# areanddee/Sharding-the-Sphere-Fall-2025-JAX-DevLab-Examples

Hardware: AMD Instinct MI355X
Metric: cell-updates/sec (whole node) at C96 (higher is better)
Workload: dtype fp64; 1 GPU; global_batch=1, seq_len=55296, parallelism=spatial tiles: 24 tiles over 1 GPU(s), auto partition, N=96, tiles_per_edge=2, integrator=ssprk3, backend=hip, comm=none, steps_per_launch=6, fused_block=16, graph_replayed_steps=0, direct_launch_steps=1662, kernel_launches=277, eager_steps=0

## Files before the change

### sharding-the-sphere-fall-2025-jax-devlab-examples_amd/ops/build.py

```python
from __future__ import annotations

import argparse
import os
import subprocess
import sys

HERE = os.path.dirname(os.path.abspath(__file__))
CSRC = os.path.join(HERE, "csrc")
LIB = os.path.join(HERE, "libstsp.so")
SOURCES = ["stage_kernel.hip", "march_kernel.hip", "march3_kernel.hip", "swe_tracer_stage.hip", "fused_step.hip", "derived_kernel.hip", "latlon_kernel.hip", "points_kernel.hip", "spectra_kernel.hip", "synth_kernel.hip", "tt_kernels.hip", "tt_persist.hip", "runtime.cpp"]
HEADERS = ["stsp_kernels.h", "stage_common.h", "xg_ring.h", "xg_codec.h", "march_common.h", "tt_common.h", "runtime.h", "rccl_abi.h"]
ARCH = os.environ.get("STSP_OFFLOAD_ARCH", "gfx950")
VARIANT_FLAGS = {"": [], "diag": ["-DSTSP_STAMPS"],
                 "unfused": ["-DSTSP_FUSE_FACES=0"], "pe0": ["-DSTSP_PE_WAVE=0"],
                 "ownw0": ["-DSTSP_OWN_SKIP0=0"], "w9": ["-DSTSP_W10=0"], "swsqrt": ["-DSTSP_HW_SQRT=0"],
                 "selslope": ["-DSTSP_SIGN_SLOPE=0"], "wpe6": ["-DSTSP_WPE=6"], "wpe7": ["-DSTSP_WPE=7"],
                 "fp_alledge": ["-DSTSP_FPROBE_ALLEDGE=1"],
                 "xgfence": ["-DSTSP_XG_FENCE=1"],
                 "hrt0": ["-DSTSP_FUSED_TAIL_OWN=0", "-DSTSP_FUSED_POLL2=0", "-DSTSP_FUSED_RF_MINB=1000"],
                 "hrt1": ["-DSTSP_FUSED_POLL2=0", "-DSTSP_FUSED_RF_MINB=1000"],
                 "hrt12": ["-DSTSP_FUSED_RF_MINB=1000"]}


def lib_for(variant: str = "") -> str:
    return LIB if not variant else os.path.join(HERE, f"libstsp_{variant}.so")


def _hipcc() -> str:
    for c in (os.environ.get("HIPCC"), "/opt/rocm/bin/hipcc", "hipcc"):
        if c and (os.path.exists(c) or c == "hipcc"):
            return c
    raise RuntimeError("hipcc not found")


def needs_build(variant: str = "") -> bool:
    lib = lib_for(variant)
    if not os.path.exists(lib):
        return True
    t = os.path.getmtime(lib)
    for f in SOURCES + HEADERS:
        p = os.path.join(CSRC, f)
        if os.path.exists(p) and os.path.getmtime(p) > t:
            return True
    return False


def _obj_dir(variant: str) -> str:
    return os.path.join(HERE, "_obj", variant or "prod")


def build(force: bool = False, verbose: bool = False, variant: str = "") -> str:
    lib = lib_for(variant)
    if not force and not needs_build(variant):
        return lib
# ... 56 lines not shown
```

### sharding-the-sphere-fall-2025-jax-devlab-examples_amd/ops/csrc/fused_step.hip

```cpp
#include "stage_common.h"

#include <type_traits>


#ifndef STSP_FPROBE_ALLEDGE
#define STSP_FPROBE_ALLEDGE 0
#endif
#ifndef STSP_XG_FENCE
#define STSP_XG_FENCE 0
#endif
#ifndef STSP_FUSED_TAGH
#define STSP_FUSED_TAGH 1
#endif
#ifndef STSP_FUSED_TAIL_OWN
#define STSP_FUSED_TAIL_OWN 1
#endif
#ifndef STSP_FUSED_POLL2
#define STSP_FUSED_POLL2 1
#endif
#ifndef STSP_FUSED_RF_MINB
#define STSP_FUSED_RF_MINB 12
#endif

namespace {

constexpr int CT_INTS = 16, CT_FLAGS = 12, CG_VALS = 8;

template <int NS, int B>
struct FD {
  static constexpr int R = 2 * NS;
  static constexpr int W = B + 2 * R;
  static constexpr int WS = W + 1;
  static constexpr int GMAX = 160;
  static constexpr int GB = W * WS;
  static constexpr int WW = GB + GMAX;
  static constexpr int L1 = R - 2 * (NS - 1);
  static constexpr int H1 = B + 4 * (NS - 1);
  static constexpr int NFX = H1 * (H1 + 1);
  static constexpr int NFL = 2 * NFX;
  static constexpr int NU = H1 * H1;
  static constexpr int NT = NU <= 768 ? 768 : 1024;
  static_assert(NU <= NT && W * W <= 2 * NT, "owner threads for every updated cell");
  static constexpr int NTAIL = W * W > NT ? W * W - NT : 0;
  static constexpr int NTO = STSP_FUSED_TAIL_OWN ? B * B : NT - NU;
  static constexpr int TPT = NTAIL ? (NTAIL + NTO - 1) / NTO : 1;
  static_assert(GMAX <= NT, "one fix-up thread per ghost entry");
  static_assert(2 * (B + 4 * (NS - 2)) * (B + 4 * (NS - 2) + 1) <= 32 * 64 && 2 * H1 * (H1 + 1) <= 32 * 64 + 64 * 64,
                "face passes per stage fit the 32-entry pass table");
  static constexpr int CMAX = 32;
};

__device__ __forceinline__ int fregion(int X, int Y, int N) {
  const bool inx = (unsigned)X < (unsigned)N, iny = (unsigned)Y < (unsigned)N;
  if (inx) return iny ? 0 : (Y < 0 ? 3 : 4);
  return iny ? (X < 0 ? 1 : 2) : -1;
}

__host__ __device__ __forceinline__ constexpr void annulus(int t, int lo, int L, int w, int& u, int& v) {
  if (t < w * L) {
    u = lo + t % L; v = lo + t / L;
    return;
  }
  t -= w * L;
  if (t < w * L) {
    u = lo + t % L; v = lo + L - w + t / L;
    return;
  }
  t -= w * L;
  const int r = t / (2 * w), c = t - r * 2 * w;
  v = lo + w + r;
  u = c < w ? lo + c : lo + L - 2 * w + c;
}

template <int NS, int B>
__host__ __device__ __forceinline__ constexpr void owner_cell(int t, int& u, int& v) {
  using D = FD<NS, B>;
  constexpr int R = D::R;
  if (t < B * B) {
    u = R + t % B; v = R + t / B;
    return;
  }
  int done = B * B;
#pragma unroll
  for (int k = 1; k <= NS; ++k) {
    const int L = B + 4 * k;
    const int n = L * L - (L - 4) * (L - 4);
    if (t < done + n) {
      annulus(t - done, R - 2 * k, L, 2, u, v);
      return;
    }
    done += n;
  }
  u = -1; v = -1;
}

template <int NS, int B>
__host__ __device__ __forceinline__ constexpr int tail_index(int tid, int k) {
  using D = FD<NS, B>;
  if (!D::NTAIL || k >= D::TPT) return -1;
  const int first = STSP_FUSED_TAIL_OWN ? 0 : D::NU;
  if (tid < first || tid >= first + D::NTO) return -1;
  const int idx = D::NT + (tid - first) + k * D::NTO;
  return idx < D::W * D::W ? idx : -1;
}

template <int NS, int B>
constexpr bool window_covered_once() {
  using D = FD<NS, B>;
  constexpr int W = D::W;
  int cnt[W * W] = {};
  for (int t = 0; t < D::NT; ++t) {
    int idx[1 + D::TPT] = {};
    idx[0] = t < W * W ? t : -1;
    for (int k = 0; k < D::TPT; ++k) idx[1 + k] = tail_index<NS, B>(t, k);
    for (int k = 0; k <= D::TPT; ++k) {
      if (idx[k] < 0) continue;
      if (k > 0 && idx[k] < D::NT) return false;
      int u = -1, v = -1;
      owner_cell<NS, B>(idx[k], u, v);
      if (u < 0 || u >= W || v < 0 || v >= W) return false;
      ++cnt[v * W + u];
    }
  }
  for (int c = 0; c < W * W; ++c)
    if (cnt[c] != 1) return false;
  return true;
}

template <typename T>
struct FArgs {
  const T* Q;
  T* out;
  const int* src;
  const int* org;
  const T* len;
  const T* nrm;
  const T* tane;
  const T* crec;
  const T* lxt;
  const T* gbt;
  unsigned long long frames;
  const unsigned long long* code;
  const int* gtab;
  const T* gw;
  const int* ctab;
  const T* cgf;
  const int* ccnt;
  const int* push;
  const int* cpush;
  int G, C, nblocks, n, N, S, mg, pw;
  int links[6];
  int local_src;
  unsigned mdiv_n;
  T a0[4], a1[4], a2[4];
  T dt, g, omega2;
  int ring, K;
  const unsigned long long* recv;
  T* const* peer_ring;
  const int* xpush;
  int* epoch;
// ... 97 lines not shown
  if (fr & 64) xi = -xi;
  if (fr & 128) xj = -xj;
  if (fr & 256) xn = -xn;
  o0 = ai == 0 ? xi : (aj == 0 ? xj : xn);
  o1 = ai == 1 ? xi : (aj == 1 ? xj : xn);
  o2 = ai == 2 ? xi : (aj == 2 ? xj : xn);
}

template <typename T>
__device__ __forceinline__ T pair_swap(T v) {
  if constexpr (sizeof(T) == 8) {
    int2 p = __builtin_bit_cast(int2, v);
    p.x = __builtin_amdgcn_update_dpp(0, p.x, 0xB1, 0xF, 0xF, false);
    p.y = __builtin_amdgcn_update_dpp(0, p.y, 0xB1, 0xF, 0xF, false);
    return __builtin_bit_cast(T, p);
  } else {
    return __builtin_bit_cast(T, __builtin_amdgcn_update_dpp(0, __builtin_bit_cast(int, v), 0xB1, 0xF, 0xF, false));
  }
}

__device__ __forceinline__ int sel5(int r, int v0, int v1, int v2, int v3, int v4) {
  return r == 0 ? v0 : r == 1 ? v1 : r == 2 ? v2 : r == 3 ? v3 : v4;
}

__device__ __forceinline__ int ncode(unsigned long long c, int side) {
  return (int)(short)(unsigned short)(c >> (16 * side));
}

template <typename T, int LIM, int NS, int B, bool XG, bool MULTI>
__global__ __launch_bounds__((FD<NS, B>::NT)) void fused_step_kernel(FArgs<T> a) {
  using D = FD<NS, B>;
  constexpr int W = D::W, WS = D::WS, WW = D::WW, GB = D::GB, R = D::R, L1 = D::L1, H1 = D::H1;
  constexpr int NFX = D::NFX, NFL = D::NFL, NT = D::NT;
  static_assert(window_covered_once<NS, B>(), "owner and tail cells cover the window exactly once");
  constexpr bool RING_FIRST = B >= STSP_FUSED_RF_MINB;
  constexpr bool PFN = sizeof(T) == 4 || B <= 16;
  constexpr int NRG = PFN ? 1 : 5;
  constexpr int NN = 2 * NRG * 3 * (W + 1);
  __shared__ T s_w[5 * WW];
  __shared__ T s_fl[4][NFL];
  __shared__ T s_len[NFL];
  __shared__ T s_nrm[2][NRG][3][W + 1];
  __shared__ T s_nrmf[PFN ? 3 * NFL : 1];
  constexpr int CS = W + 1;
  __shared__ unsigned long long s_code[W * CS];
  __shared__ short s_gs[D::GMAX][2];
  __shared__ T s_gt[D::GMAX];
  __shared__ int s_ct[D::CMAX][CT_INTS];
  __shared__ T s_cg[D::CMAX][CG_VALS];
  constexpr int NX2 = NS > 1 ? (B + 4 * (NS - 2)) * (B + 4 * (NS - 2)) : 1;
  __shared__ T s_x[4][NX2];
  __shared__ int s_gdone;

  const int tid = threadIdx.x;
  const int bid = xcd_remap(blockIdx.x, a.nblocks);
  const int N = a.N;
  const int* og = a.org + bid * 4;
  const int X0 = og[0], Y0 = og[1], tile = og[2], ow = og[3];
  const int xo = ow & 0xFFF, yo = (ow >> 12) & 0xFFF, flags = (ow >> 24) & 0x1F;
  const bool edge = (flags & 0x1E) != 0;
  const int ngw = edge ? (a.G + 63) >> 6 : 0;
  int gbase = 0;
  int gtarget = 0;
  if (tid == 0) s_gdone = 0;
  const T* wf = &s_w[0];
  FSTAMP(0);
  FSTAMP_RT(14);
  if (a.stamps && (tid & 63) == 0) {
    unsigned long long* sp = a.stamps + ((long)bid * 16 + (tid >> 6)) * FST_W;
    sp[16] = __builtin_amdgcn_s_getreg((31 << 11) | 4);
    sp[17] = __builtin_amdgcn_s_getreg((31 << 11) | 20);
    sp[18] = blockIdx.x;
  }

  int u = -1, v = -1;
  const bool owner = tid < W * W;
  if (owner) owner_cell<NS, B>(tid, u, v);
  const int wi = v * WS + u;
  int xe = 0;
  const int nsteps = MULTI ? a.nsteps : 1;
  const bool epoch_on = XG || MULTI;
  const bool tagh = STSP_FUSED_TAGH && MULTI && a.hx != nullptr;
  const bool pcell = MULTI && !XG && !tagh && a.pidx != nullptr;
  if (epoch_on) xe = a.epoch[bid];
  const int n = a.n;
  const int face0 = (int)((unsigned)ow >> 29);
  auto cell_src = [&](int cu, int cv, int& g_, int& I_, int& J_) -> int {
    if (!window_cell(face0, X0 + cu, Y0 + cv, N, a.links, g_, I_, J_)) return -1;
    if (a.local_src) {
      const int t = N / n;
      const int ti = a.mdiv_n ? (int)__umulhi((unsigned)I_, a.mdiv_n) : I_ / n;
      const int tj = a.mdiv_n ? (int)__umulhi((unsigned)J_, a.mdiv_n) : J_ / n;
      return (((g_ * t + tj) * t + ti) * a.pw + (J_ - tj * n) + a.mg) * a.pw + (I_ - ti * n) + a.mg;
    }
    return a.src[(long)bid * W * W + cv * W + cu];
  };
  int cg_ = 0, cI = 0, cJ = 0;
  const int src = owner ? cell_src(u, v, cg_, cI, cJ) : -1;
  unsigned long long cdv = 0;
  int gs0 = 0, gs1 = 0;
  T gtv = T(0);
  int ncor = 0;
  int ctv[CT_INTS];
  T cgv[CG_VALS];
  if (edge) {
    if (owner) cdv = a.code[(long)bid * W * W + v * W + u];
    if (tid < a.G) {
      gs0 = a.gtab[((long)bid * a.G + tid) * 2];
      gs1 = a.gtab[((long)bid * a.G + tid) * 2 + 1];
// ... 28 lines not shown
      const int r = yf ? jj / H1 : jj / (H1 + 1), c = yf ? jj - r * H1 : jj - r * (H1 + 1);
      const int li = yf ? (X0 + L1 + c) * (N + 1) + Y0 + L1 + r : (Y0 + L1 + r) * (N + 1) + X0 + L1 + c;
      lnv[k] = j < NFL ? a.lxt[li] : T(0);
    }
  } else {
#pragma unroll
    for (int k = 0; k < LPT; ++k) {
      const int j = tid + k * NT;
      lnv[k] = j < NFL ? a.len[(long)bid * NFL + j] : T(0);
    }
  }
  T nrv = T(0);
  const bool nr_ld = flags == 1 ? tid < 2 * (W + 1) : (!PFN && tid < NN);
  T nrv2 = T(0);
  if (nr_ld) {
    if (flags == 1) nrv = a.tane[(tid < W + 1 ? X0 + tid : Y0 + tid - (W + 1))];
    else nrv = a.nrm[(long)bid * NN + tid];
  }
  static_assert(NN <= 2 * NT, "line-normal table: two values per thread at most");
  if (!PFN && NN > NT && flags != 1 && tid + NT < NN) nrv2 = a.nrm[(long)bid * NN + tid + NT];
  constexpr int NPF = PFN ? (3 * NFL + NT - 1) / NT : 1;
  T nfv[NPF];
  if (PFN && flags != 1) {
#pragma unroll
    for (int k = 0; k < NPF; ++k) {
      const int j = tid + k * NT;
      nfv[k] = j < 3 * NFL ? a.nrmf[(long)bid * 3 * NFL + j] : T(0);
    }
  }
  T Q[4];
  T iA = T(0), r0 = T(0), r1 = T(0), r2 = T(0), gb0 = T(0), gb1 = T(0), gb2 = T(0), S0 = T(0), S1 = T(0),
    S2 = T(0);
  const bool loaded = src >= 0 || (XG && src <= -2);
  const bool in1 = tid < (B + 4 * (NS - 1)) * (B + 4 * (NS - 1));
  auto load_state_of = [&](int src, T (&Q)[4], const T* Qin, int xe_) {
    const bool loaded = src >= 0 || (XG && src <= -2);
    if (XG && src <= -2) {
      unsigned long long gr[HX<T>::W];
      const XgRec r = ring_slot_record<HX<T>>(a.recv, a.ring, xg_in_slot(xe_), -2 - src);
      fused_wait<HX<T>, XG_RING_SCOPE, STSP_XG_FENCE != 0>(r, xg_in_tag(xe_), a.err, a.timeout_ticks, gr, [&] {
        fused_fail(a.err, 1u, bid, xe_, -2 - src, (int)HX<T>::tag_of(gr[0]));
      });
      HX<T>::unpack(gr, Q);
    } else if (loaded) {
      const unsigned S = (unsigned)a.S;
      unsigned so = (unsigned)src;
      asm volatile("" : "+v"(so));
#pragma unroll
      for (int f = 0; f < 4; ++f) Q[f] = ld_state<true>(o32(Qin, so + f * S));
    } else {
#pragma unroll
      for (int f = 0; f < 4; ++f) Q[f] = T(0);
    }
  };
  auto hx_record = [&](unsigned so, int slot) -> XgRec {
    const unsigned S = (unsigned)a.S;
    return {(gu64*)a.hx + (size_t)slot * HX<T>::W * S + so, (long)S};
  };
  auto load_tagged = [&](int src_, T (&q)[4], int xe_) {
#if STSP_FUSED_TAIL_OWN
    asm volatile("" : "+v"(src_));
#endif
    unsigned long long gr[HX<T>::W];
    const XgRec r = hx_record((unsigned)src_, xe_ & 1);
    fused_wait<HX<T>, XG_LOCAL_SCOPE>(r, xg_in_tag(xe_), a.err, a.timeout_ticks, gr, [&] {
      fused_fail(a.err, 2u, bid, xe_, src_, (int)HX<T>::tag_of(gr[0]));
    });
// ... 286 lines not shown
      tail_load(buf[it & 1], xe, tq);
      if (tid >= B * B) {
        load_state(buf[it & 1], xe);
        enter_cell();
      }
    }
    tail_put(tq);
    FSTAMP(19);
    __syncthreads();
  }
  FSTAMP(2);

#pragma unroll
  for (int s = 0; s < NS; ++s) {
    const int lo = R - 2 * (NS - 1 - s), hi = W - lo;
    const int nr = hi - lo, nl = nr + 1, nx = nr * nl;
    if (edge) {
      const int ge = tid - gbase;
      if (ge >= 0 && ge < a.G) {
        const int i0 = s_gs[ge][0], i1 = s_gs[ge][1];
        const T t = s_gt[ge];
#pragma unroll
        for (int f = 0; f < 4; ++f) {
          const T x0 = wf[f * WW + i0], x1 = wf[f * WW + i1];
          s_w[f * WW + GB + ge] = x0 + t * (x1 - x0);
        }
      }
      if (ge >= 0 && ge < ngw * 64 && (tid & 63) == 0) {
        asm volatile("s_waitcnt lgkmcnt(0)" ::: "memory");
        __hip_atomic_fetch_add(&s_gdone, 1, __ATOMIC_RELEASE, __HIP_MEMORY_SCOPE_WORKGROUP);
      }
      gtarget += ngw;
    }
    const int nax = s == 0 ? NOX : nx;
    const int ntask = 2 * nax;
    unsigned m = pmask[s];
    for (int first = (ncor && wv == 0) ? 1 : 0; first || m;) {
      int task;
      bool nearp = false;
      if (first) {
        task = (tid & 63) - 64;
        first = 0;
      } else {
        const int pp = __builtin_ctz(m);
        task = pp * 64 + (tid & 63);
        nearp = (nmask[s] >> pp) & 1u;
        m &= m - 1u;
      }
      if (task >= ntask) continue;
      if (task >= 0) {
        const int tf = task;
        const bool ax = tf >= nax;
        const int t2 = ax ? tf - nax : tf;
        int fu, fv, k, p;
        if (s == 0) {
          outer_face(t2, k, p);
        } else {
          const int c = t2 / nr, r = t2 - c * nr;
          k = lo + c; p = lo + r;
        }
        if (!ax) { fv = p; fu = k; }
        else { fu = p; fv = k; }
        if (edge || STSP_FPROBE_ALLEDGE) {
          if (PFN && !nearp) face(ax, fu, fv, k, std::integral_constant<int, 1>{});
          else face(ax, fu, fv, k, std::integral_constant<int, 2>{});
        } else {
          face(ax, fu, fv, k, std::integral_constant<int, 0>{});
        }
      } else {
        const int lane = tid & 63, j = lane >> 1, q = lane & 1;
        const bool live = j < ncor;
        T fvq[4], ccq[5];
#pragma unroll
        for (int f = 0; f < 4; ++f) fvq[f] = T(0);
#pragma unroll
        for (int f = 0; f < 5; ++f) ccq[f] = T(0);
        int fl_ = 0;
        if (live) {
          const int* ct = s_ct[j];
          fl_ = ct[CT_FLAGS];
          const int ic = ct[5 * q], a0 = ct[5 * q + 1], a1 = ct[5 * q + 2], n0 = ct[5 * q + 3], n1 = ct[5 * q + 4];
          const bool plus = (fl_ >> (4 + q)) & 1, ai = (fl_ >> (2 * q)) & 1, ni = (fl_ >> (2 * q + 1)) & 1;
          const T ta = s_cg[j][4 + 2 * q], tn = s_cg[j][5 + 2 * q];
#pragma unroll
          for (int f = 0; f < 5; ++f) ccq[f] = wf[f * WW + ic];
#pragma unroll
          for (int f = 0; f < 4; ++f) {
            const T c0 = ccq[f];
            const T xa = wf[f * WW + a0], xn = wf[f * WW + n0];
            const T across = ai ? xa + ta * (wf[f * WW + a1] - xa) : xa;
            const T inward = ni ? xn + tn * (wf[f * WW + n1] - xn) : xn;
            fvq[f] = plus ? c0 + half_slope<LIM>(c0 - inward, across - c0)
                          : c0 - half_slope<LIM>(c0 - across, inward - c0);
          }
        }
        T fvp[4], ccp[5];
#pragma unroll
        for (int f = 0; f < 4; ++f) fvp[f] = pair_swap(fvq[f]);
#pragma unroll
        for (int f = 0; f < 5; ++f) ccp[f] = pair_swap(ccq[f]);
        if (live && q == 0) {
          T fl[4];
          swe_flux<T>(fvq, fvp, ccq, ccp, s_cg[j][0], s_cg[j][1], s_cg[j][2], s_cg[j][3], a.g, fl);
          const int fc = s_ct[j][10], fd = s_ct[j][11];
          const bool pc = (fl_ >> 4) & 1, pd = (fl_ >> 5) & 1;
#pragma unroll
          for (int f = 0; f < 4; ++f) {
            if (fc >= 0) s_fl[f][fc] = pc ? fl[f] : -fl[f];
            if (fd >= 0) s_fl[f][fd] = pd ? -fl[f] : fl[f];
          }
        }
      }
    }
    FSTAMP(10 + s);
    __syncthreads();
    FSTAMP(3 + 2 * s);
    const bool upd = loaded && tid < nr * nr;
    if (upd) {
      const int xw = (v - L1) * (H1 + 1) + (u - L1), xe_ = xw + 1;
      const int ys = NFX + (v - L1) * H1 + (u - L1), yn = ys + H1;
      T dq[4];
#pragma unroll
      for (int f = 0; f < 4; ++f) dq[f] = -((s_fl[f][xe_] - s_fl[f][xw]) + (s_fl[f][yn] - s_fl[f][ys])) * iA;
      const T h = Q[0];
      const T fcor = a.omega2 * r2;
      const T cor[3] = {r1 * Q[3] - r2 * Q[2], r2 * Q[1] - r0 * Q[3], r0 * Q[2] - r1 * Q[1]};
      const T pb = T(0.5) * a.g * h * h * iA, gh = a.g * h;
      const T gbv[3] = {gb0, gb1, gb2}, Sv[3] = {S0, S1, S2};
#pragma unroll
      for (int k = 0; k < 3; ++k) dq[1 + k] += -fcor * cor[k] + pb * Sv[k] - gh * gbv[k];
      const T c0 = a.a0[s], c1 = a.a1[s], c2 = a.a2[s] * a.dt;
      T o[4];
#pragma unroll
      for (int f = 0; f < 4; ++f) {
        T base = c1 * Q[f];
        if (c0 != T(0)) base += c0 * s_x[f][tid];
        o[f] = c2 * dq[f] + base;
      }
      const T dd = o[1] * r0 + o[2] * r1 + o[3] * r2;
      o[1] -= dd * r0; o[2] -= dd * r1; o[3] -= dd * r2;
#pragma unroll
      for (int f = 0; f < 4; ++f) Q[f] = o[f];
      if (s + 1 < NS) put(Q);
    }
    if (s + 1 < NS) __syncthreads();
    FSTAMP(4 + 2 * s);
  }

  T* const Out = buf[(it + 1) & 1];
  const bool last = it + 1 == nsteps;
// ... 185 lines not shown
  return -5;
}

template <typename T>
__global__ __launch_bounds__(256) void fused_prime_kernel(const T* __restrict__ q, int S,
                                                          const int* __restrict__ src, const int* __restrict__ code,
                                                          int nent, T* const* peer_ring, int ring, int epoch) {
  const int i = blockIdx.x * blockDim.x + threadIdx.x;
  if (i < nent) {
    xg_prime_record<HX<T>, 4>(q, S, src[i], code[i], peer_ring, ring, epoch);
  }
  __threadfence_system();
}

extern "C" int stsp_fused_record_words(int dtype) { return dtype == 1 ? HX<double>::W : HX<float>::W; }

extern "C" int stsp_fused_prime_launch(int dtype, const void* q, int S, const int* src, const int* code, int nent,
                                       void* const* peer_ring, int ring, int epoch, hipStream_t stream) {
  if (nent <= 0) return 0;
  const dim3 grid((nent + 255) / 256), block(256);
  if (dtype == 1)
    hipLaunchKernelGGL(fused_prime_kernel<double>, grid, block, 0, stream, (const double*)q, S, src, code, nent,
                       (double* const*)peer_ring, ring, epoch);
  else if (dtype == 0)
    hipLaunchKernelGGL(fused_prime_kernel<float>, grid, block, 0, stream, (const float*)q, S, src, code, nent,
                       (float* const*)peer_ring, ring, epoch);
  else
    return -4;
  return (int)hipGetLastError();
}

extern "C" int stsp_fused_tagh(void) { return STSP_FUSED_TAGH; }

extern "C" int stsp_fused_limits(int* gmax, int* cmax) {
  *gmax = FD<3, 16>::GMAX;
  *cmax = FD<3, 16>::CMAX;
  return 0;
}
```

### sharding-the-sphere-fall-2025-jax-devlab-examples_amd/ops/fused.py

```python
from __future__ import annotations

import hashlib
import os
from dataclasses import dataclass
from typing import Dict, List, Optional, Tuple

import numpy as np
import torch

from ..models.base import panel_edge_tables
from ..parallel.layout import TileLayout, ghost_xy
from ..parallel.topology import neighbor_cells


def native_stream(device) -> int:
    from .native import current_stream_handle
    return current_stream_handle(device)

REG_P, REG_W, REG_E, REG_S, REG_N = 0, 1, 2, 3, 4
NREG = 5
SIDE_VEC = ((-1, 0), (1, 0), (0, -1), (0, 1))
NG_PLR = 2


# ... 704 lines not shown
        e.time += e.dt
        e.step_count += 1



FUSED_BLOCKS = (6, 8, 12, 16, 18, 20)


def rank_cus(device) -> int:
    import os
    cus = torch.cuda.get_device_properties(device).multi_processor_count
    if os.environ.get("STSP_SHARE_GPU") == "1":
        cus = max(1, cus // max(1, int(os.environ.get("WORLD_SIZE", "1"))))
    return cus


def fused_block(n: int, tiles: Optional[int] = None, cus: Optional[int] = None) -> Optional[int]:
    fits = [B for B in FUSED_BLOCKS if n % B == 0]
    if not fits:
        return None
    if tiles is not None and cus is not None:
        for B in fits:
            if tiles * (n // B) ** 2 <= cus:
                return B
    return fits[-1]



def fused_threads(B: int, ns: int = 3) -> int:
    h1 = B + 4 * (ns - 1)
    return 768 if h1 * h1 <= 768 else 1024


def stage_face_counts(B: int, ns: int = 3) -> List[int]:
    h1 = B + 4 * (ns - 1)
    nil = B - 3
    out = [2 * (h1 * (h1 + 1) - nil * B)]
    for s in range(1, ns):
        nr = B + 4 * (ns - 1 - s)
        out.append(2 * nr * (nr + 1))
    return out


PASS_SLOTS = 32


def pass_schedule(B: int, ncorner: np.ndarray, edge: np.ndarray, G: int, ns: int = 3,
                  weights: Optional[str] = None) -> np.ndarray:
    import os
    weights = weights or os.environ.get("STSP_FUSED_SCHED", "5:1")
    nt = fused_threads(B, ns)
    nw = nt // 64
    counts = stage_face_counts(B, ns)
    nb = len(ncorner)
    out = np.zeros((nb, ns, PASS_SLOTS), dtype=np.uint8)
    ngw = -(-G // 64) if G > 0 else 0
    cache = {}
    for b in range(nb):
        cw = 1 if ncorner[b] > 0 else 0
        gw = ngw if edge[b] else 0
        key = (cw, gw)
        if key not in cache:
            tab = np.zeros((ns, PASS_SLOTS), dtype=np.uint8)
            for s, nt_s in enumerate(counts):
                npass = -(-nt_s // 64)
                assert npass <= PASS_SLOTS
                if weights == "legacy":
                    first = nw - cw
                    for p in range(npass):
                        tab[s, p] = p + cw if p < first else cw + gw + (p - first) % (nw - cw - gw)
                    continue
                wc, wg = (int(x) for x in weights.split(":"))
                wl = [0] * nw
                if cw:
                    wl[0] += wc
                for w in range(cw, cw + gw):
                    wl[w] += wg
                for p in range(npass):
                    gl = [sum(wl[w] for w in range(g, nw, 4)) for g in range(4)]
                    g = min(range(4), key=lambda g_: (gl[g_], g_))
                    w = min(range(g, nw, 4), key=lambda w_: (wl[w_], w_))
                    tab[s, p] = w
                    wl[w] += 4
            cache[key] = tab
        out[b] = cache[key]
    return out


def pass_masks(B: int, sched: np.ndarray, ns: int = 3, near: Optional[np.ndarray] = None) -> np.ndarray:
    counts = stage_face_counts(B, ns)
    nb = sched.shape[0]
    m = np.zeros((nb, ns, 17), dtype=np.uint32)
    for s_, cnt in enumerate(counts):
        for p in range(-(-cnt // 64)):
            w = sched[:, s_, p].astype(np.int64)
            m[np.arange(nb), s_, w] |= np.uint32(1 << p)
    if near is not None:
        m[:, :, 16] = near
    return m


def stage_face_coords(B: int, ns: int = 3) -> List[Tuple[np.ndarray, np.ndarray, np.ndarray]]:
    d = FusedDims.make(B, ns)
    R, W, L1, H1 = d.R, d.W, d.L1, d.H1
    nil = B - 3
    ol0 = R + 2 - L1
    ol1 = (W - L1) - (R + B - 1) + 1
    nr1, nor = H1, H1 - B
    noa = (ol0 + ol1) * nr1
    nox = noa + nil * nor
    out = []
    for s_ in range(ns):
        if s_ == 0:
            nax = nox
            t = np.arange(nax)
            k = np.empty(nax, np.int64)
            p = np.empty(nax, np.int64)
            a = t < noa
            li, r = np.divmod(t[a], nr1)
            k[a] = np.where(li < ol0, L1 + li, R + B - 1 + (li - ol0))
            p[a] = L1 + r
            t2 = t[~a] - noa
            li, r = np.divmod(t2, nor)
            k[~a] = R + 2 + li
            p[~a] = np.where(r < R - L1, L1 + r, R + B + (r - (R - L1)))
        else:
            lo = R - 2 * (ns - 1 - s_)
            nr = W - 2 * lo
            nax = nr * (nr + 1)
            c, r = np.divmod(np.arange(nax), nr)
            k, p = lo + c, lo + r
        out.append((np.concatenate([np.zeros(nax, np.int64), np.ones(nax, np.int64)]),
                    np.concatenate([k, k]), np.concatenate([p, p])))
    return out


def near_pass_masks(B: int, org: np.ndarray, flags: np.ndarray, N: int, ns: int = 3) -> np.ndarray:
    nb = org.shape[0]
    out = np.zeros((nb, ns), dtype=np.uint32)
    coords = stage_face_coords(B, ns)
    far = -1000
    X0, Y0 = org[:, 0].astype(np.int64), org[:, 1].astype(np.int64)
    kx0 = np.where(flags & 2, -X0, far)
    kx1 = np.where(flags & 4, N - X0, far)
    ky0 = np.where(flags & 8, -Y0, far)
    ky1 = np.where(flags & 16, N - Y0, far)
    for s_, (ax, k, _) in enumerate(coords):
        e0 = np.where(ax[None, :] == 1, ky0[:, None], kx0[:, None])
        e1 = np.where(ax[None, :] == 1, ky1[:, None], kx1[:, None])
        kk = k[None, :]
        near = ((kk - e0 + 1 >= 0) & (kk - e0 + 1 <= 2)) | ((kk - e1 + 1 >= 0) & (kk - e1 + 1 <= 2))
        npass = -(-near.shape[1] // 64)
        for p in range(npass):
            hit = near[:, 64 * p:64 * (p + 1)].any(1)
            out[hit, s_] |= np.uint32(1 << p)
    return out


def face_normals(P: "FusedPlan", flags: np.ndarray) -> np.ndarray:
    d = P.d
    H1, L1 = d.H1, d.L1
    nfx = d.nfx
    nfl = 2 * nfx
    j = np.arange(nfl)
    yf = j >= nfx
    jj = np.where(yf, j - nfx, j)
    r = np.where(yf, jj // H1, jj // (H1 + 1))
    c = np.where(yf, jj - r * H1, jj - r * (H1 + 1))
    fu = L1 + c
    fv = L1 + r
    k = np.where(yf, fv, fu)
    lu = fu - np.where(yf, 0, 1)
    lv = fv - np.where(yf, 1, 0)
# ... 44 lines not shown
        if why:
            raise RuntimeError(why)
        if B is None:
            cus = None
            if engine.device.type == "cuda":
                cus = rank_cus(engine.device)
            B = fused_block(engine.plan.n, len(engine.plan.tiles), cus)
        e = engine
        self.e = e
        self.group = group
        self.lib = native.require_native()
        self._launch_fn = self.lib.stsp_fused_launch
        world = e.layout.num_ranks
        self.world = world
        X = None
        if world > 1 or e.layout.loopback:
            X = FusedExchangePlan(e.layout, e.grid, B, ns=3)
            P = X.plans[e.rank]
        else:
            P = FusedPlan(e.layout, e.rank, e.grid, B=B, ns=3)
            P.src[~P.need[:, 0]] = -1
        self.plan = P
        d = P.d
        W, WS, nb = d.W, d.W + 1, P.nb
        dev, dt = e.device, e.dtype
        gmax, cmax = ctypes_limits(self.lib)
        G, C = P.gtab.shape[1], P.ctab.shape[1]
        if G > gmax or C > cmax:
            raise RuntimeError(f"fused step: {G} ghost entries / {C} corner faces exceed the kernel's {gmax} / {cmax}")
        S = e.plan.S
        nring = X.ring_slots if X is not None else 0
        assert P.src.shape == (nb, W * W) and int(P.src.max()) < S and int(P.src.min()) >= -2 - (nring - 1)
        assert (P.src[P.need[:, 0]] != -1).all()
        nfl = 2 * d.nfx
        ld = lambda s_: (s_ // W) * WS + s_ % W
        for b in range(nb):
            k = int(P.gcnt[b])
            assert (P.gtab[b, :k, 2:4] >= 0).all() and (P.gtab[b, :k, 2:4] < W * W).all()
            for j in range(int(P.ccnt[b])):
                assert -1 <= P.ctab[b, j, 4] < nfl and -1 <= P.ctab[b, j, 5] < nfl
        assert int(P.gidx.max()) < G
        code = neighbour_codes(P)
        gpair = np.zeros((nb, G, 2), dtype=np.int32)
        gpair[..., 0] = ld(P.gtab[..., 2])
        gpair[..., 1] = ld(P.gtab[..., 3])
        ct, cgw = corner_tables(P, code, gpair)
        org = P.org.copy()
        for b in range(nb):
            regs = set(int(x) for x in np.unique(P.reg[b]) if x >= 0)
            flags = sum(1 << r for r in regs)
            li, rem = divmod(b, P.nbx * P.nby)
            yb, xb = divmod(rem, P.nbx)
            face = e.layout.tile_origin(e.plan.tiles[li])[0]
            org[b, 3] = np.int32(np.uint32((xb * B) | ((yb * B) << 12) | (flags << 24) | (face << 29)).view(np.int32))
        kg = kernel_geometry(e.layout, e.grid)
        self.frames = [int(x) for x in kg["frames"]]
        t = lambda a, ty=dt: torch.as_tensor(np.ascontiguousarray(a), dtype=ty, device=dev)
        self.tens = {
            "len": t(np.concatenate([P.lx.reshape(nb, -1), P.ly.reshape(nb, -1)], 1)),
            "nrm": t(np.ascontiguousarray(np.moveaxis(P.nrm, -1, -2))),
            "tane": t(kg["tane"]), "crec": t(kg["crec"]), "lxt": t(kg["lxt"]),
            "src": t(P.src, torch.int32), "org": t(org, torch.int32),
            "code": t(code.view(np.int64), torch.int64), "gtab": t(gpair, torch.int32), "gw": t(P.gt),
            "ctab": t(ct, torch.int32), "cgf": t(cgw), "ccnt": t(P.ccnt, torch.int32),
            "push": torch.as_tensor(e.plan.push_map, dtype=torch.int32, device=dev).contiguous(),
            "cpush": torch.as_tensor(e.plan.corner_push, dtype=torch.int32, device=dev).contiguous(),
# ... 9 lines not shown
            for li, tid in enumerate(e.plan.tiles):
                f, I0, J0 = L_.tile_origin(tid)
                gbn[li, ng:ng + n, ng:ng + n, :3] = rec_g[L_.global_flat(f, I0 + ii, J0 + jj), 4:7]
            gbn = gbn.reshape(-1, 4)
            if X is not None:
                rg = np.zeros((len(X.need_remote[e.rank]), 4))
                rg[:, :3] = rec_g[X.need_remote[e.rank], 4:7]
                gbn = np.concatenate([gbn, rg], 0)
            self.tens["gbt"] = t(gbn)
        assert int(e.plan.push_map.max(initial=-1)) < S and int(e.plan.corner_push.max(initial=-1)) < S
        self.dcode = native.dtype_code(dt)
        self.mem = None
        self.tens["epoch"] = torch.zeros(nb, dtype=torch.int32, device=dev)
        self.handoff = handoff_mode(B, multi_rank=X is not None)
        if self.handoff == "tag" and not read_relation_symmetric(P):
            if os.environ.get("STSP_FUSED_HANDOFF") == "tag":
                raise RuntimeError("tagged hand-off needs a symmetric block read relation")
            self.handoff = "epoch"
        if self.handoff == "tag" and not int(self.lib.stsp_fused_tagh()):
            if os.environ.get("STSP_FUSED_HANDOFF") == "tag":
                raise RuntimeError("STSP_FUSED_HANDOFF=tag needs a library built with STSP_FUSED_TAGH=1")
            self.handoff = "epoch"
        if self.handoff == "tag":
            words = 5 if e.dtype == torch.float64 else 4
            self.tens["hx"] = torch.zeros(2 * words * e.plan.S, dtype=torch.int64, device=dev)
        self.tens["err"] = torch.zeros(8, dtype=torch.int32, device=dev)
        prod = producer_table(P)
        self.tens["prod"] = torch.as_tensor(prod, dtype=torch.int32, device=dev).contiguous()
        self.poll = poll_mode() if (X is None and self.handoff == "epoch" and read_relation_symmetric(P)) \
            else "block"
        if self.poll == "cell":
            self.tens["pidx"] = torch.as_tensor(cell_producer_index(P, prod), device=dev).contiguous()
        edge_b = np.array([any(int(x) > 0 for x in np.unique(P.reg[b])) for b in range(nb)])
        sched = pass_schedule(B, np.asarray(P.ccnt), edge_b, G)
        assert int(sched.max()) < fused_threads(B) // 64
        flg = (org[:, 3].view(np.uint32) >> 24) & 0x1F
        near = near_pass_masks(B, P.org, flg.astype(np.int64), e.layout.N)
        self.tens["sched"] = torch.as_tensor(pass_masks(B, sched, near=near).view(np.int32), device=dev).contiguous()
        self.tens["nrmf"] = t(face_normals(P, flg.astype(np.int64)))
        self.timeout_ticks = int(timeout_s * 1e8)
        if X is not None:
            self._setup_exchange(X, timeout_s)
        self.descs = [self._desc(0, 1), self._desc(1, 0)]
        self._multi = {}
        self._multi_ptrs = {}
        if X is not None:
            self.prime()

    def _setup_exchange(self, X, timeout_s: float) -> None:
        from .xgmi import IpcRing, _declare, refuse_if_forced
        refuse_if_forced()
        e = self.e
        L = _declare(self.lib)
        self._xlib = L
        self.slots = int(L.stsp_xg_slots())
        self.ring = X.ring_slots * int(self.lib.stsp_fused_record_words(self.dcode))
        xpush, psrc, pcode = X.producer(e.rank)
        assert psrc.size == 0 or int(psrc.max()) < e.plan.S
        peers = sorted(set(int(c) >> XG_SLOT_BITS for c in pcode.tolist())
                       | set(int(x) for x in np.unique(np.asarray(e.layout.owner)[
                           e.layout.locate(X.need_remote[e.rank])[0]]).tolist()))
        self.mem = IpcRing(L, e.device, self.world, e.rank, peers, self.slots * self.ring * 8, self.group)
        pr = np.zeros(32, dtype=np.int64)
        for p, b in self.mem.bases.items():
            pr[p] = b
        dev = e.device
        self.tens.update({
            "peer_ring": torch.as_tensor(pr, device=dev),
            "xpush": torch.as_tensor(xpush, dtype=torch.int32, device=dev).contiguous(),
            "prime_src": torch.as_tensor(psrc, dtype=torch.int32, device=dev),
            "prime_code": torch.as_tensor(pcode, dtype=torch.int32, device=dev),
# ... 369 lines not shown
```

### sharding-the-sphere-fall-2025-jax-devlab-examples_amd/ops/native.py

```python
from __future__ import annotations

import ctypes
import os
import threading

import torch

from . import build as _build

_LIB = None
_LOCK = threading.Lock()


class StageDesc(ctypes.Structure):
    _fields_ = [
        ("X", ctypes.c_void_p), ("Q", ctypes.c_void_p), ("acc_in", ctypes.c_void_p),
        ("out", ctypes.c_void_p), ("acc_out", ctypes.c_void_p), ("recv", ctypes.c_void_p),
        ("gmap", ctypes.c_void_p), ("push", ctypes.c_void_p), ("blocks", ctypes.c_void_p),
        ("invA", ctypes.c_void_p), ("ex", ctypes.c_void_p), ("ey", ctypes.c_void_p),
        ("mx", ctypes.c_void_p), ("my", ctypes.c_void_p), ("cgeo", ctypes.c_void_p),
        ("ntile", ctypes.c_int), ("n", ctypes.c_int), ("S", ctypes.c_int), ("mg", ctypes.c_int), ("pw", ctypes.c_int),
        ("nblocks", ctypes.c_int), ("limiter", ctypes.c_int), ("remote", ctypes.c_int),
        ("a0", ctypes.c_double), ("a1", ctypes.c_double), ("a2", ctypes.c_double),
        ("c0", ctypes.c_double), ("c1", ctypes.c_double), ("c2", ctypes.c_double), ("dt", ctypes.c_double),
# ... 115 lines not shown
    ("stsp_synth_launch", [_P(SynthDesc), _VP], SynthDesc, ("stsp_synth_desc_size", ())),
]


def lib_path() -> str:
    return _build.lib_for(os.environ.get("STSP_VARIANT", ""))


def load(build_if_missing: bool = True):
    global _LIB
    with _LOCK:
        if _LIB is not None:
            return _LIB
        variant = os.environ.get("STSP_VARIANT", "")
        path = _build.lib_for(variant)
        if build_if_missing and _build.needs_build(variant):
            try:
                _build.build(variant=variant)
            except Exception:
                if not os.path.exists(path):
                    raise
        L = ctypes.CDLL(path, mode=ctypes.RTLD_GLOBAL)
        vp, ci, cl = ctypes.c_void_p, ctypes.c_int, ctypes.c_long
        L.stsp_pack_launch.argtypes = [ci, vp, ci, ci, vp, ci, vp, vp]
        L.stsp_pack_launch.restype = ci
        L.stsp_copy_index_launch.argtypes = [ci, vp, vp, vp, vp, ci, ci, cl, cl, vp]
        L.stsp_copy_index_launch.restype = ci
        L.stsp_dpp_probe.argtypes = [vp, vp, vp, vp]
        L.stsp_dpp_probe.restype = ci
        L.stsp_fused_limits.argtypes = [ctypes.POINTER(ci), ctypes.POINTER(ci)]
        L.stsp_fused_limits.restype = ci
        L.stsp_fused_tagh.argtypes = []
        L.stsp_fused_tagh.restype = ci
        L.stsp_fused_record_words.argtypes = [ci]
        L.stsp_fused_record_words.restype = ci
        L.stsp_fused_prime_launch.argtypes = [ci, vp, ci, vp, vp, ci, vp, ci, ci, vp]
        L.stsp_fused_prime_launch.restype = ci
        for launch, argtypes, cls, (query, args) in DESCRIPTORS:
            fn, size = getattr(L, launch), getattr(L, query)
            fn.argtypes, fn.restype = argtypes, ci
            size.argtypes, size.restype = [ci] * len(args), ci
            if size(*args) != ctypes.sizeof(cls):
                raise RuntimeError(f"{cls.__name__}: ctypes mirror is {ctypes.sizeof(cls)} bytes, "
                                   f"the library's {size(*args)} (stale libstsp.so?)")
        _declare_runtime(L)
        _declare_tt(L)
        L.stsp_schedule_spin.argtypes = [ci]
        L.stsp_schedule_spin.restype = ci
        L.stsp_device_flags.argtypes = []
        L.stsp_device_flags.restype = ci
        _LIB = L
        return L


def _declare_runtime(L):
    vp, ci, cd = ctypes.c_void_p, ctypes.c_int, ctypes.c_double
    if not hasattr(L, "stsp_rt_create"):
        return
    L.stsp_rt_create.argtypes = [vp]
    L.stsp_rt_create.restype = vp
    L.stsp_rt_destroy.argtypes = [vp]
    L.stsp_rt_destroy.restype = None
    L.stsp_rt_run.argtypes = [vp, ci]
    L.stsp_rt_run.restype = ci
    L.stsp_rt_set_dt.argtypes = [vp, cd]
    L.stsp_rt_set_dt.restype = ci
# ... 125 lines not shown
```

Baseline: 4.887 billion cell-updates/s.

## Shrink fused multi-stage halo from square to diamond cone shape

The fused SSPRK3 step kernel used to recompute every cell of a square halo window at each stage. It now limits owner cells and face-flux tasks to a diamond (L1-distance) cone around the block, which is the region the stencil actually depends on. This drops the redundant corner computation and face fluxes. The cost is more complex index arithmetic in owner_cell and cone_face, plus host-side schedule and mask changes, guarded by compile-time coverage checks.

After: 4.874 billion cell-updates/s. About the same (-0.3%).

```diff
diff --git a/sharding-the-sphere-fall-2025-jax-devlab-examples_amd/ops/build.py b/sharding-the-sphere-fall-2025-jax-devlab-examples_amd/ops/build.py
--- a/sharding-the-sphere-fall-2025-jax-devlab-examples_amd/ops/build.py
+++ b/sharding-the-sphere-fall-2025-jax-devlab-examples_amd/ops/build.py
@@ -19,7 +19,8 @@
                  "xgfence": ["-DSTSP_XG_FENCE=1"],
                  "hrt0": ["-DSTSP_FUSED_TAIL_OWN=0", "-DSTSP_FUSED_POLL2=0", "-DSTSP_FUSED_RF_MINB=1000"],
                  "hrt1": ["-DSTSP_FUSED_POLL2=0", "-DSTSP_FUSED_RF_MINB=1000"],
-                 "hrt12": ["-DSTSP_FUSED_RF_MINB=1000"]}
+                 "hrt12": ["-DSTSP_FUSED_RF_MINB=1000"],
+                 "cone0": ["-DSTSP_FUSED_CONE=0"]}
 
 
 def lib_for(variant: str = "") -> str:
diff --git a/sharding-the-sphere-fall-2025-jax-devlab-examples_amd/ops/csrc/fused_step.hip b/sharding-the-sphere-fall-2025-jax-devlab-examples_amd/ops/csrc/fused_step.hip
--- a/sharding-the-sphere-fall-2025-jax-devlab-examples_amd/ops/csrc/fused_step.hip
+++ b/sharding-the-sphere-fall-2025-jax-devlab-examples_amd/ops/csrc/fused_step.hip
@@ -21,10 +21,25 @@
 #ifndef STSP_FUSED_RF_MINB
 #define STSP_FUSED_RF_MINB 12
 #endif
+#ifndef STSP_FUSED_CONE
+#define STSP_FUSED_CONE 1
+#endif
 
 namespace {
 
 constexpr int CT_INTS = 16, CT_FLAGS = 12, CG_VALS = 8;
+
+__host__ __device__ constexpr bool in_shape(int NS, int B, int s, int u, int v) {
+  const int R = 2 * NS, m = 2 * (NS - s);
+  if (u < 0 || v < 0 || u >= B + 2 * R || v >= B + 2 * R) return false;
+  const int du = u < R ? R - u : (u >= R + B ? u - (R + B - 1) : 0);
+  const int dv = v < R ? R - v : (v >= R + B ? v - (R + B - 1) : 0);
+  return STSP_FUSED_CONE ? du + dv <= m : (du <= m && dv <= m);
+}
+__host__ __device__ constexpr int shape_cells(int NS, int B, int s) {
+  const int m = 2 * (NS - s);
+  return (B + 2 * m) * (B + 2 * m) - (STSP_FUSED_CONE ? 2 * m * (m + 1) : 0);
+}
 
 template <int NS, int B>
 struct FD {
@@ -38,10 +53,11 @@
   static constexpr int H1 = B + 4 * (NS - 1);
   static constexpr int NFX = H1 * (H1 + 1);
   static constexpr int NFL = 2 * NFX;
-  static constexpr int NU = H1 * H1;
-  static constexpr int NT = NU <= 768 ? 768 : 1024;
-  static_assert(NU <= NT && W * W <= 2 * NT, "owner threads for every updated cell");
-  static constexpr int NTAIL = W * W > NT ? W * W - NT : 0;
+  static constexpr int NC = shape_cells(NS, B, 0);
+  static constexpr int NU = shape_cells(NS, B, 1);
+  static constexpr int NT = H1 * H1 <= 768 ? 768 : 1024;
+  static_assert(NU <= NT && NC <= 2 * NT, "owner threads for every updated cell");
+  static constexpr int NTAIL = NC > NT ? NC - NT : 0;
   static constexpr int NTO = STSP_FUSED_TAIL_OWN ? B * B : NT - NU;
   static constexpr int TPT = NTAIL ? (NTAIL + NTO - 1) / NTO : 1;
   static_assert(GMAX <= NT, "one fix-up thread per ghost entry");
@@ -81,6 +97,33 @@
     return;
   }
   int done = B * B;
+#if STSP_FUSED_CONE
+#pragma unroll
+  for (int j = 1; j <= NS; ++j) {
+    const int n = 8 * B + 16 * j - 12;
+    if (t < done + n) {
+      int q = t - done;
+      const int lo = R - 2 * j, hi = R + B - 1 + 2 * j;
+      if (q < 2 * (2 * B + 2)) {
+        const bool bot = q >= 2 * B + 2;
+        if (bot) q -= 2 * B + 2;
+        const int in = q >= B ? 1 : 0;
+        if (in) q -= B;
+        u = R - in + q;
+        v = bot ? hi - in : lo + in;
+      } else {
+        q -= 2 * (2 * B + 2);
+        const int r = q >> 2, c = q & 3;
+        v = lo + 2 + r;
+        const int dv = v < R ? R - v : (v >= R + B ? v - (R + B - 1) : 0);
+        const int du = 2 * j - dv - ((c == 1 || c == 2) ? 1 : 0);
+        u = c < 2 ? R - du : R + B - 1 + du;
+      }
+      return;
+    }
+    done += n;
+  }
+#else
 #pragma unroll
   for (int k = 1; k <= NS; ++k) {
     const int L = B + 4 * k;
@@ -91,6 +134,7 @@
     }
     done += n;
   }
+#endif
   u = -1; v = -1;
 }
 
@@ -101,31 +145,84 @@
   const int first = STSP_FUSED_TAIL_OWN ? 0 : D::NU;
   if (tid < first || tid >= first + D::NTO) return -1;
   const int idx = D::NT + (tid - first) + k * D::NTO;
-  return idx < D::W * D::W ? idx : -1;
+  return idx < D::NC ? idx : -1;
 }
 
 template <int NS, int B>
-constexpr bool window_covered_once() {
+constexpr bool shape_covered_once() {
   using D = FD<NS, B>;
   constexpr int W = D::W;
   int cnt[W * W] = {};
   for (int t = 0; t < D::NT; ++t) {
     int idx[1 + D::TPT] = {};
-    idx[0] = t < W * W ? t : -1;
+    idx[0] = t < D::NC ? t : -1;
     for (int k = 0; k < D::TPT; ++k) idx[1 + k] = tail_index<NS, B>(t, k);
     for (int k = 0; k <= D::TPT; ++k) {
       if (idx[k] < 0) continue;
       if (k > 0 && idx[k] < D::NT) return false;
       int u = -1, v = -1;
       owner_cell<NS, B>(idx[k], u, v);
-      if (u < 0 || u >= W || v < 0 || v >= W) return false;
+      if (!in_shape(NS, B, 0, u, v)) return false;
+      for (int s = 1; s <= NS; ++s)
+        if ((idx[k] < shape_cells(NS, B, s)) != in_shape(NS, B, s, u, v)) return false;
       ++cnt[v * W + u];
     }
   }
   for (int c = 0; c < W * W; ++c)
-    if (cnt[c] != 1) return false;
+    if (cnt[c] != (in_shape(NS, B, 0, c % W, c / W) ? 1 : 0)) return false;
   return true;
 }
+
+#if STSP_FUSED_CONE
+template <int NS, int B>
+__host__ __device__ constexpr int cone_nax(int s) {
+  const int m = 2 * (NS - 1 - s), pa = m * B + m * (m - 1);
+  return s == 0 ? 2 * pa + 4 * (B + 2 * m) + (B - 3) * 2 * m : 2 * pa + (B + 1) * (B + 2 * m);
+}
+template <int NS, int B>
+__host__ __device__ __forceinline__ constexpr void cone_face(int s, int t, int& k, int& p) {
+  constexpr int R = 2 * NS;
+  const int m = 2 * (NS - 1 - s), lo = R - m;
+  const int nmid = s == 0 ? 4 : B + 1;
+  const int pa = m * B + m * (m - 1), lm = B + 2 * m, pm = nmid * lm;
+  if (s == 0 && t >= 2 * pa + pm) {
+    const int t2 = t - (2 * pa + pm), li = t2 / (2 * m > 0 ? 2 * m : 1), r = t2 - li * 2 * m;
+    k = R + 2 + li;
+    p = r < m ? lo + r : R + B + (r - m);
+    return;
+  }
+  const bool desc = t >= pa + pm, mid = t >= pa && !desc;
+  const int x = desc ? 2 * pa + pm - 1 - t : t;
+  int j = 0, off = 0;
+#pragma unroll
+  for (int q = 1; q < 2 * (NS - 1); ++q)
+    if (q < m && x >= q * B + q * (q - 1)) { j = q; off = q * B + q * (q - 1); }
+  const int tm = t - pa, lq = tm / lm;
+  const int li = mid ? m + lq : (desc ? 2 * m + nmid - 1 - j : j);
+  p = mid ? lo + (tm - lq * lm) : R - j + (x - off);
+  k = s == 0 && li >= m + 2 ? R + B - 1 + (li - (m + 2)) : lo + li;
+}
+template <int NS, int B>
+constexpr bool cone_faces_once() {
+  constexpr int R = 2 * NS, W = B + 2 * R;
+  for (int s = 0; s < NS; ++s) {
+    int cnt[(W + 1) * W] = {};
+    for (int t = 0; t < cone_nax<NS, B>(s); ++t) {
+      int k = -1, p = -1;
+      cone_face<NS, B>(s, t, k, p);
+      if (k < 0 || k > W || p < 0 || p >= W) return false;
+      ++cnt[k * W + p];
+    }
+    for (int k = 0; k <= W; ++k)
+      for (int p = 0; p < W; ++p) {
+        const bool inner = s == 0 && k >= R + 2 && k <= R + B - 2 && p >= R && p < R + B;
+        const bool want = !inner && (in_shape(NS, B, s + 1, k - 1, p) || in_shape(NS, B, s + 1, k, p));
+        if (cnt[k * W + p] != (want ? 1 : 0)) return false;
+      }
+  }
+  return true;
+}
+#endif
 
 template <typename T>
 struct FArgs {
@@ -289,7 +386,10 @@
   using D = FD<NS, B>;
   constexpr int W = D::W, WS = D::WS, WW = D::WW, GB = D::GB, R = D::R, L1 = D::L1, H1 = D::H1;
   constexpr int NFX = D::NFX, NFL = D::NFL, NT = D::NT;
-  static_assert(window_covered_once<NS, B>(), "owner and tail cells cover the window exactly once");
+  static_assert(shape_covered_once<NS, B>(), "owner and tail cells cover the step's shape exactly once");
+#if STSP_FUSED_CONE
+  static_assert(cone_faces_once<NS, B>(), "face tasks cover the faces of each stage's shape exactly once");
+#endif
   constexpr bool RING_FIRST = B >= STSP_FUSED_RF_MINB;
   constexpr bool PFN = sizeof(T) == 4 || B <= 16;
   constexpr int NRG = PFN ? 1 : 5;
@@ -305,7 +405,7 @@
   __shared__ T s_gt[D::GMAX];
   __shared__ int s_ct[D::CMAX][CT_INTS];
   __shared__ T s_cg[D::CMAX][CG_VALS];
-  constexpr int NX2 = NS > 1 ? (B + 4 * (NS - 2)) * (B + 4 * (NS - 2)) : 1;
+  constexpr int NX2 = NS > 1 ? shape_cells(NS, B, 2) : 1;
   __shared__ T s_x[4][NX2];
   __shared__ int s_gdone;
 
@@ -331,7 +431,7 @@
   }
 
   int u = -1, v = -1;
-  const bool owner = tid < W * W;
+  const bool owner = tid < D::NC;
   if (owner) owner_cell<NS, B>(tid, u, v);
   const int wi = v * WS + u;
   int xe = 0;
@@ -426,7 +526,7 @@
   T iA = T(0), r0 = T(0), r1 = T(0), r2 = T(0), gb0 = T(0), gb1 = T(0), gb2 = T(0), S0 = T(0), S1 = T(0),
     S2 = T(0);
   const bool loaded = src >= 0 || (XG && src <= -2);
-  const bool in1 = tid < (B + 4 * (NS - 1)) * (B + 4 * (NS - 1));
+  const bool in1 = tid < D::NU;
   auto load_state_of = [&](int src, T (&Q)[4], const T* Qin, int xe_) {
     const bool loaded = src >= 0 || (XG && src <= -2);
     if (XG && src <= -2) {
@@ -779,7 +879,11 @@
       }
       gtarget += ngw;
     }
+#if STSP_FUSED_CONE
+    const int nax = cone_nax<NS, B>(s);
+#else
     const int nax = s == 0 ? NOX : nx;
+#endif
     const int ntask = 2 * nax;
     unsigned m = pmask[s];
     for (int first = (ncor && wv == 0) ? 1 : 0; first || m;) {
@@ -800,12 +904,16 @@
         const bool ax = tf >= nax;
         const int t2 = ax ? tf - nax : tf;
         int fu, fv, k, p;
+#if STSP_FUSED_CONE
+        cone_face<NS, B>(s, t2, k, p);
+#else
         if (s == 0) {
           outer_face(t2, k, p);
         } else {
           const int c = t2 / nr, r = t2 - c * nr;
           k = lo + c; p = lo + r;
         }
+#endif
         if (!ax) { fv = p; fu = k; }
         else { fu = p; fv = k; }
         if (edge || STSP_FPROBE_ALLEDGE) {
@@ -862,7 +970,7 @@
     FSTAMP(10 + s);
     __syncthreads();
     FSTAMP(3 + 2 * s);
-    const bool upd = loaded && tid < nr * nr;
+    const bool upd = loaded && tid < shape_cells(NS, B, s + 1);
     if (upd) {
       const int xw = (v - L1) * (H1 + 1) + (u - L1), xe_ = xw + 1;
       const int ys = NFX + (v - L1) * H1 + (u - L1), yn = ys + H1;
@@ -1114,6 +1222,8 @@
 
 extern "C" int stsp_fused_tagh(void) { return STSP_FUSED_TAGH; }
 
+extern "C" int stsp_fused_cone(void) { return STSP_FUSED_CONE; }
+
 extern "C" int stsp_fused_limits(int* gmax, int* cmax) {
   *gmax = FD<3, 16>::GMAX;
   *cmax = FD<3, 16>::CMAX;
diff --git a/sharding-the-sphere-fall-2025-jax-devlab-examples_amd/ops/fused.py b/sharding-the-sphere-fall-2025-jax-devlab-examples_amd/ops/fused.py
--- a/sharding-the-sphere-fall-2025-jax-devlab-examples_amd/ops/fused.py
+++ b/sharding-the-sphere-fall-2025-jax-devlab-examples_amd/ops/fused.py
@@ -760,7 +760,59 @@
     return 768 if h1 * h1 <= 768 else 1024
 
 
-def stage_face_counts(B: int, ns: int = 3) -> List[int]:
+def cone_shape(B: int, ns: int = 3, cone: bool = True) -> np.ndarray:
+    d = FusedDims.make(B, ns)
+    x = np.arange(d.W)
+    dist = np.maximum(np.maximum(d.R - x, x - (d.R + B - 1)), 0)
+    du, dv = dist[None, :], dist[:, None]
+    out = np.zeros((ns + 1, d.W, d.W), dtype=bool)
+    for s in range(ns + 1):
+        m = NG_PLR * (ns - s)
+        out[s] = (du + dv <= m) if cone else ((du <= m) & (dv <= m))
+    return out
+
+
+def _cone_axis_tasks(B: int, ns: int, s_: int) -> Tuple[np.ndarray, np.ndarray]:
+    R = NG_PLR * ns
+    m = NG_PLR * (ns - 1 - s_)
+    lo = R - m
+    nmid = 4 if s_ == 0 else B + 1
+    pa, lm = m * B + m * (m - 1), B + 2 * m
+    pm = nmid * lm
+    nax = 2 * pa + pm + ((B - 3) * 2 * m if s_ == 0 else 0)
+    t = np.arange(nax)
+    k = np.empty(nax, np.int64)
+    p = np.empty(nax, np.int64)
+    inner = t >= 2 * pa + pm
+    if inner.any():
+        li, r = np.divmod(t[inner] - (2 * pa + pm), 2 * m)
+        k[inner] = R + 2 + li
+        p[inner] = np.where(r < m, lo + r, R + B + (r - m))
+    w = ~inner
+    tw = t[w]
+    desc = tw >= pa + pm
+    mid = (tw >= pa) & ~desc
+    x = np.where(desc, 2 * pa + pm - 1 - tw, tw)
+    j = np.zeros_like(tw)
+    off = np.zeros_like(tw)
+    for q in range(1, m):
+        hit = x >= q * B + q * (q - 1)
+        j[hit], off[hit] = q, q * B + q * (q - 1)
+    lq, rm = np.divmod(tw - pa, lm)
+    li = np.where(mid, m + lq, np.where(desc, 2 * m + nmid - 1 - j, j))
+    p[w] = np.where(mid, lo + rm, R - j + (x - off))
+    k[w] = np.where((li >= m + 2), R + B - 1 + (li - (m + 2)), lo + li) if s_ == 0 else lo + li
+    return k, p
+
+
+def stage_face_counts(B: int, ns: int = 3, cone: bool = True) -> List[int]:
+    if cone:
+        out = []
+        for s in range(ns):
+            m = NG_PLR * (ns - 1 - s)
+            pa = m * B + m * (m - 1)
+            out.append(2 * (2 * pa + (4 * (B + 2 * m) + (B - 3) * 2 * m if s == 0 else (B + 1) * (B + 2 * m))))
+        return out
     h1 = B + 4 * (ns - 1)
     nil = B - 3
     out = [2 * (h1 * (h1 + 1) - nil * B)]
@@ -774,12 +826,12 @@
 
 
 def pass_schedule(B: int, ncorner: np.ndarray, edge: np.ndarray, G: int, ns: int = 3,
-                  weights: Optional[str] = None) -> np.ndarray:
+                  weights: Optional[str] = None, cone: bool = True) -> np.ndarray:
     import os
     weights = weights or os.environ.get("STSP_FUSED_SCHED", "5:1")
     nt = fused_threads(B, ns)
     nw = nt // 64
-    counts = stage_face_counts(B, ns)
+    counts = stage_face_counts(B, ns, cone)
     nb = len(ncorner)
     out = np.zeros((nb, ns, PASS_SLOTS), dtype=np.uint8)
     ngw = -(-G // 64) if G > 0 else 0
@@ -815,8 +867,9 @@
     return out
 
 
-def pass_masks(B: int, sched: np.ndarray, ns: int = 3, near: Optional[np.ndarray] = None) -> np.ndarray:
-    counts = stage_face_counts(B, ns)
+def pass_masks(B: int, sched: np.ndarray, ns: int = 3, near: Optional[np.ndarray] = None,
+               cone: bool = True) -> np.ndarray:
+    counts = stage_face_counts(B, ns, cone)
     nb = sched.shape[0]
     m = np.zeros((nb, ns, 17), dtype=np.uint32)
     for s_, cnt in enumerate(counts):
@@ -828,7 +881,15 @@
     return m
 
 
-def stage_face_coords(B: int, ns: int = 3) -> List[Tuple[np.ndarray, np.ndarray, np.ndarray]]:
+def stage_face_coords(B: int, ns: int = 3, cone: bool = True) -> List[Tuple[np.ndarray, np.ndarray, np.ndarray]]:
+    if cone:
+        out = []
+        for s_ in range(ns):
+            k, p = _cone_axis_tasks(B, ns, s_)
+            nax = len(k)
+            out.append((np.concatenate([np.zeros(nax, np.int64), np.ones(nax, np.int64)]),
+                        np.concatenate([k, k]), np.concatenate([p, p])))
+        return out
     d = FusedDims.make(B, ns)
     R, W, L1, H1 = d.R, d.W, d.L1, d.H1
     nil = B - 3
@@ -863,10 +924,11 @@
     return out
 
 
-def near_pass_masks(B: int, org: np.ndarray, flags: np.ndarray, N: int, ns: int = 3) -> np.ndarray:
+def near_pass_masks(B: int, org: np.ndarray, flags: np.ndarray, N: int, ns: int = 3,
+                    cone: bool = True) -> np.ndarray:
     nb = org.shape[0]
     out = np.zeros((nb, ns), dtype=np.uint32)
-    coords = stage_face_coords(B, ns)
+    coords = stage_face_coords(B, ns, cone)
     far = -1000
     X0, Y0 = org[:, 0].astype(np.int64), org[:, 1].astype(np.int64)
     kx0 = np.where(flags & 2, -X0, far)
@@ -977,6 +1039,13 @@
         nring = X.ring_slots if X is not None else 0
         assert P.src.shape == (nb, W * W) and int(P.src.max()) < S and int(P.src.min()) >= -2 - (nring - 1)
         assert (P.src[P.need[:, 0]] != -1).all()
+        self.cone = bool(self.lib.stsp_fused_cone()) if hasattr(self.lib, "stsp_fused_cone") else False
+        shape = cone_shape(B, 3, self.cone).reshape(d.ns + 1, W * W)
+        outside = P.need & ~shape[None]
+        if outside.any():
+            b_, s_, c_ = (int(x[0]) for x in np.nonzero(outside))
+            raise RuntimeError(f"fused step: block {b_} needs window cell ({c_ % W}, {c_ // W}) at stage {s_}, "
+                               f"outside the kernel's {'cone' if self.cone else 'square'} for B = {B}")
         nfl = 2 * d.nfx
         ld = lambda s_: (s_ // W) * WS + s_ % W
         for b in range(nb):
@@ -1052,11 +1121,12 @@
         if self.poll == "cell":
             self.tens["pidx"] = torch.as_tensor(cell_producer_index(P, prod), device=dev).contiguous()
         edge_b = np.array([any(int(x) > 0 for x in np.unique(P.reg[b])) for b in range(nb)])
-        sched = pass_schedule(B, np.asarray(P.ccnt), edge_b, G)
+        sched = pass_schedule(B, np.asarray(P.ccnt), edge_b, G, cone=self.cone)
         assert int(sched.max()) < fused_threads(B) // 64
         flg = (org[:, 3].view(np.uint32) >> 24) & 0x1F
-        near = near_pass_masks(B, P.org, flg.astype(np.int64), e.layout.N)
-        self.tens["sched"] = torch.as_tensor(pass_masks(B, sched, near=near).view(np.int32), device=dev).contiguous()
+        near = near_pass_masks(B, P.org, flg.astype(np.int64), e.layout.N, cone=self.cone)
+        self.tens["sched"] = torch.as_tensor(pass_masks(B, sched, near=near, cone=self.cone).view(np.int32),
+                                             device=dev).contiguous()
         self.tens["nrmf"] = t(face_normals(P, flg.astype(np.int64)))
         self.timeout_ticks = int(timeout_s * 1e8)
         if X is not None:
diff --git a/sharding-the-sphere-fall-2025-jax-devlab-examples_amd/ops/native.py b/sharding-the-sphere-fall-2025-jax-devlab-examples_amd/ops/native.py
--- a/sharding-the-sphere-fall-2025-jax-devlab-examples_amd/ops/native.py
+++ b/sharding-the-sphere-fall-2025-jax-devlab-examples_amd/ops/native.py
@@ -171,6 +171,9 @@
         L.stsp_fused_limits.restype = ci
         L.stsp_fused_tagh.argtypes = []
         L.stsp_fused_tagh.restype = ci
+        if hasattr(L, "stsp_fused_cone"):
+            L.stsp_fused_cone.argtypes = []
+            L.stsp_fused_cone.restype = ci
         L.stsp_fused_record_words.argtypes = [ci]
         L.stsp_fused_record_words.restype = ci
         L.stsp_fused_prime_launch.argtypes = [ci, vp, ci, vp, vp, ci, vp, ci, ci, vp]
```
